# anands-repo/hello

Hardware: AMD Instinct MI355X
Metric: candidate sites/sec (whole node) (higher is better)
Workload: dtype f32

## Files before the change

### hello_amd/csrc/engine.hip

```cpp
#include <hip/hip_runtime.h>

#include <cstdarg>
#include <cstdio>
#include <cstring>
#include <new>
#include <stdexcept>
#include <string>
#include <vector>

#include "../../include/hello_mi355x.h"
#include "kernels.h"

namespace {

thread_local std::string g_last_error;

int fail(int code, const char* fmt, ...) {
    char buf[512];
    va_list ap;
    va_start(ap, fmt);
    vsnprintf(buf, sizeof(buf), fmt, ap);
    va_end(ap);
    g_last_error = buf;
    return code;
}

// ... 108 lines not shown
    bool timed = false;
    bool profiling = false;
    std::vector<std::vector<hipEvent_t>> prof_events;
    int prof_count = 0;
    int prof_filter = 0;
    int debug_op = -1;
    DevBuf d_debug;
    size_t debug_floats = 0;
    int stamp_mode = 0;
    DevBuf d_stamps;
    int32_t stamp_layout[5] = {0, 0, 0, 0, 0};

    int32_t *roff0 = nullptr, *roff1 = nullptr, *aoff = nullptr, *site_of_allele = nullptr;
    int32_t *allele_of_read0 = nullptr, *allele_of_read1 = nullptr;
    int32_t *group_slot0 = nullptr, *group_slot1 = nullptr, *slot_off0 = nullptr, *slot_off1 = nullptr;
    hello::ReadConvPlan plan0{1, 0, 0}, plan1{1, 0, 0};
    bool wide_trunk[2] = {false, false};
    int64_t* pair_off = nullptr;
};

namespace {

long long rows_of(int domain, int32_t S, int32_t A, int64_t R0, int64_t R1) {
    switch (domain) {
        case HELLO_ROWS_READS0: return R0;
        case HELLO_ROWS_READS1: return R1;
        case HELLO_ROWS_ALLELES: return A;
        case HELLO_ROWS_SITES: return S;
    }
    return -1;
}
// ... 341 lines not shown
            delete e;
            return fail(HELLO_ERR_MODEL, "a weight block runs past the end of the blob");
        }
    }
    e->scratch.resize(desc->n_buffers);
    hipError_t err = hipMalloc((void**)&e->d_weights, nbytes);
    if (err == hipSuccess) err = hipMemcpy(e->d_weights, folded_weights, nbytes, hipMemcpyHostToDevice);
    if (err == hipSuccess) err = hipStreamCreateWithFlags(&e->own_stream, hipStreamNonBlocking);
    if (err == hipSuccess) err = hipEventCreateWithFlags(&e->ev_staged, hipEventDisableTiming);
    if (err == hipSuccess) err = hipEventCreate(&e->ev_start);
    if (err == hipSuccess) err = hipEventCreate(&e->ev_stop);
    if (err != hipSuccess) {
        hello_engine_destroy(e);
        return fail(HELLO_ERR_HIP, "engine setup failed: %s", hipGetErrorString(err));
    }
    const int n_ops = (int)e->ops.size();
    e->n_lanes = lanes.n_lanes;
    e->partial_of.assign(n_ops, -1);
    int n_partial = e->n_lanes > 1 ? 0 : 2;
    for (int i = 0; i < n_ops; ++i)
        if (e->ops[i].kind == HELLO_OP_READCONV_FUSED)
            e->partial_of[i] = e->n_lanes > 1 ? n_partial++ : (e->ops[i].seg == HELLO_SEG_READS1_TO_ALLELES ? 1 : 0);
    e->d_partial.resize(n_partial);
    if (e->n_lanes > 1) {
        auto lane_of = [&](int i) { return lane_of_op(e->ops[i]); };
        e->op_waits = std::move(lanes.op_waits);
        e->lane_tail = std::move(lanes.lane_tail);
        const std::vector<char>& read_elsewhere = lanes.read_elsewhere;
        e->op_done.assign(n_ops, nullptr);
        e->lane_streams.assign(e->n_lanes, nullptr);
// ... 156 lines not shown
    HIP_TRY(hipSetDevice(e->device));
    HIP_TRY(hipStreamSynchronize(e->last_stream ? e->last_stream : e->own_stream));
    HIP_TRY(hipMemcpy(out, e->d_debug.p, e->debug_floats * sizeof(float), hipMemcpyDeviceToHost));
    return HELLO_OK;
} catch (...) {
    return hello::exception_status("hello_engine_debug_read");
}

static int stage_batch_indices(hello_engine* e, const int32_t* rpa0, const int32_t* rpa1,
                               const int32_t* aps, int32_t S, int32_t A, int64_t R0, int64_t R1,
                               bool two_tech, hipStream_t stream) {
    const int win = hello::readconv_supports_window(e->desc.window) ? e->desc.window : 150;
    const int G = hello::readconv_reads_per_group(win);
    if ((e->wide_trunk[0] || e->wide_trunk[1]) && hello::readconv_wide_reads_per_group() != G)
        return fail(HELLO_ERR_ARG, "internal: the wide trunk's group size differs from the read convolver's");
    const hello::ReadConvPlan plan0 = e->wide_trunk[0] ? hello::readconv_wide_plan(R0) : hello::readconv_plan(R0, win);
    const hello::ReadConvPlan plan1 = !two_tech ? hello::ReadConvPlan{1, 0, 0}
                                      : e->wide_trunk[1] ? hello::readconv_wide_plan(R1) : hello::readconv_plan(R1, win);
    const int64_t n_groups0 = plan0.bulk_wgs + plan0.rest_wgs, n_groups1 = plan1.bulk_wgs + plan1.rest_wgs;
    e->plan0 = plan0;
    e->plan1 = plan1;
    size_t bytes = 0;
    auto add = [&](size_t count, size_t elem) { bytes += (count * elem + 15) & ~size_t(15); };
    add(A + 1, 4); add(A + 1, 4); add(S + 1, 4); add(A, 4);
    add(R0, 4); add(R1, 4);
    add(n_groups0 + 1, 4); add(n_groups1 + 1, 4);
    add(A + 1, 4); add(A + 1, 4);
    add(S + 1, 8);
    if (e->staged_pending) {
        HIP_TRY(hipEventSynchronize(e->ev_staged));
        e->staged_pending = false;
    }
    if (e->h_csr.ensure(bytes)) return fail(HELLO_ERR_HIP, "pinned allocation of %zu bytes failed", bytes);
    if (bytes > e->d_csr.cap) {
        HIP_TRY(hipStreamSynchronize(stream));
        if (e->d_csr.ensure(bytes)) return fail(HELLO_ERR_HIP, "device allocation of %zu bytes failed", bytes);
    }
    char* hc = (char*)e->h_csr.p;
    char* hbase = hc;
    int32_t* h_roff0 = carve<int32_t>(hc, A + 1);
    int32_t* h_roff1 = carve<int32_t>(hc, A + 1);
    int32_t* h_aoff = carve<int32_t>(hc, S + 1);
    int32_t* h_soa = carve<int32_t>(hc, A);
    int32_t* h_aor0 = carve<int32_t>(hc, R0);
    int32_t* h_aor1 = carve<int32_t>(hc, R1);
    int32_t* h_gs0 = carve<int32_t>(hc, n_groups0 + 1);
    int32_t* h_gs1 = carve<int32_t>(hc, n_groups1 + 1);
    int32_t* h_so0 = carve<int32_t>(hc, A + 1);
    int32_t* h_so1 = carve<int32_t>(hc, A + 1);
    int64_t* h_poff = carve<int64_t>(hc, S + 1);

    auto build_reads = [&](const int32_t* rpa, int64_t R, int32_t* roff, int32_t* aor, int32_t* gslot,
                           int32_t* soff, const hello::ReadConvPlan& plan, const char* which) -> int {
        int64_t acc = 0;
        for (int32_t a = 0; a < A; ++a) {
            if (rpa[a] <= 0)
                return fail(HELLO_ERR_SHAPE, "%s[%d] = %d: every allele needs >= 1 read (dummy zero read)",
                            which, a, rpa[a]);
            roff[a] = (int32_t)acc;
            for (int32_t r = 0; r < rpa[a]; ++r) {
                if (acc + r < R) aor[acc + r] = a;
            }
            acc += rpa[a];
            if (acc > R) return fail(HELLO_ERR_SHAPE, "sum(%s) exceeds n_reads = %lld", which, (long long)R);
        }
        roff[A] = (int32_t)acc;
        if (acc != R)
            return fail(HELLO_ERR_SHAPE, "sum(%s) = %lld != n_reads = %lld", which, (long long)acc, (long long)R);
        const int64_t n_wgs = plan.bulk_wgs + plan.rest_wgs;
        const int64_t bulk_reads = plan.rest_wgs ? plan.bulk_wgs * plan.groups_per_wg * G : R;
        for (int32_t a = 0; a <= A; ++a) soff[a] = 0;
        int64_t slot = 0;
        for (int64_t w = 0; w < n_wgs; ++w) {
            int64_t r_lo, r_hi;
            if (w < plan.bulk_wgs) {
                r_lo = w * plan.groups_per_wg * G;
                r_hi = r_lo + (int64_t)plan.groups_per_wg * G;
                if (r_hi > bulk_reads) r_hi = bulk_reads;
            } else {
                r_lo = bulk_reads + (w - plan.bulk_wgs) * G;
                r_hi = r_lo + G < R ? r_lo + G : R;
            }
            if (r_lo >= r_hi) return fail(HELLO_ERR_ARG, "internal: empty workgroup in the read-convolver plan");
            gslot[w] = (int32_t)slot;
            const int32_t first = aor[r_lo], last = aor[r_hi - 1];
            for (int32_t a = first; a <= last; ++a) soff[a + 1] += 1;
            slot += (last - first + 1);
        }
        gslot[n_wgs] = (int32_t)slot;
        int64_t s = 0;
        for (int32_t a = 0; a < A; ++a) {
            const int32_t count = soff[a + 1];
            soff[a] = (int32_t)s;
            s += count;
        }
        soff[A] = (int32_t)s;
        if (s != slot) return fail(HELLO_ERR_ARG, "internal: slot accounting mismatch");
        return 0;
    };
    if (int rc = build_reads(rpa0, R0, h_roff0, h_aor0, h_gs0, h_so0, plan0, "reads_per_allele0")) return rc;
    if (two_tech) {
        if (int rc = build_reads(rpa1, R1, h_roff1, h_aor1, h_gs1, h_so1, plan1, "reads_per_allele1")) return rc;
    } else {
        h_gs1[0] = 0;
    }
    int64_t acc = 0, pacc = 0;
    for (int32_t s = 0; s < S; ++s) {
        if (aps[s] <= 0) return fail(HELLO_ERR_SHAPE, "alleles_per_site[%d] = %d", s, aps[s]);
        h_aoff[s] = (int32_t)acc;
        h_poff[s] = pacc;
        for (int32_t k = 0; k < aps[s] && acc + k < A; ++k) h_soa[acc + k] = s;
        acc += aps[s];
        pacc += (int64_t)aps[s] * (aps[s] + 1) / 2;
        if (acc > A) return fail(HELLO_ERR_SHAPE, "sum(alleles_per_site) exceeds n_alleles = %d", A);
    }
    h_aoff[S] = (int32_t)acc;
    h_poff[S] = pacc;
    if (acc != A) return fail(HELLO_ERR_SHAPE, "sum(alleles_per_site) = %lld != n_alleles = %d", (long long)acc, A);

    HIP_TRY(hipMemcpyAsync(e->d_csr.p, hbase, bytes, hipMemcpyHostToDevice, stream));
    HIP_TRY(hipEventRecord(e->ev_staged, stream));
    e->staged_pending = true;
    char* dbase = (char*)e->d_csr.p;
    auto dev = [&](void* hp) { return dbase + ((char*)hp - hbase); };
    e->roff0 = (int32_t*)dev(h_roff0);
    e->roff1 = (int32_t*)dev(h_roff1);
    e->aoff = (int32_t*)dev(h_aoff);
    e->site_of_allele = (int32_t*)dev(h_soa);
    e->allele_of_read0 = (int32_t*)dev(h_aor0);
    e->allele_of_read1 = (int32_t*)dev(h_aor1);
    e->group_slot0 = (int32_t*)dev(h_gs0);
    e->group_slot1 = (int32_t*)dev(h_gs1);
    e->slot_off0 = (int32_t*)dev(h_so0);
    e->slot_off1 = (int32_t*)dev(h_so1);
    e->pair_off = (int64_t*)dev(h_poff);
    return 0;
}

int hello_engine_forward(hello_engine* e, const uint8_t* reads0, const int32_t* rpa0,
                         const uint8_t* reads1, const int32_t* rpa1, const int32_t* aps,
                         const uint8_t* ref_onehot, int32_t S, int32_t A, int64_t R0, int64_t R1,
                         float* logits, float* meta, float* posteriors, int32_t flags, void* hip_stream) try {
    if (!e) return fail(HELLO_ERR_ARG, "engine is NULL");
    const hello_model_desc& d = e->desc;
    const bool two_tech = d.channels1 > 0;
    if (S <= 0 || A <= 0 || R0 <= 0) return fail(HELLO_ERR_ARG, "empty batch (S=%d A=%d R0=%lld)", S, A, (long long)R0);
    if (A < S) return fail(HELLO_ERR_SHAPE, "n_alleles %d < n_sites %d", A, S);
// ... 258 lines not shown
                a.w = e->d_weights + o.w_off;
                a.partial = (float*)e->d_partial[e->partial_of[op_index]].p;
                a.allele_of_read = t1 ? e->allele_of_read1 : e->allele_of_read0;
                a.slot_of_group = t1 ? e->group_slot1 : e->group_slot0;
                a.n_reads = t1 ? R1 : R0;
                a.window = d.window;
                a.softplus = (o.flags & HELLO_FLAG_SOFTPLUS) ? 1 : 0;
                a.extra_blocks = o.k;
                a.winograd = (o.flags & HELLO_FLAG_WINOGRAD) ? 1 : 0;
                a.bf16x3 = (o.flags & HELLO_FLAG_BF16X3) ? ((o.flags & HELLO_FLAG_BF16X3_32) ? 2 : 1) : 0;
                const bool wide = o.cout == 128;
                if ((size_t)o.w_off + (wide ? hello::readconv_wide_weight_floats() : hello::readconv_weight_floats(o.k, a.winograd, d.window)) +
                        (a.bf16x3 ? hello::readconv_bf16x3_extra_floats(o.k) : 0) > e->n_weight_floats)
                    return fail(HELLO_ERR_MODEL, "op %d: fused read-convolver weight block truncated", op_index);
                {
                    const hello::ReadConvPlan& plan = t1 ? e->plan1 : e->plan0;
                    const int G = hello::readconv_reads_per_group(d.window);
                    const long long total = a.n_reads;
                    const long long bulk_reads = plan.rest_wgs ? plan.bulk_wgs * plan.groups_per_wg * G : total;
                    a.groups_per_wg = plan.groups_per_wg;
                    a.n_reads = bulk_reads;
                    int32_t stamp_lay[5] = {0, 0, 0, 0, 0};
                    const int stamp_waves = hello::readconv_stamp_waves();
                    if ((e->stamp_mode & 1) && !t1 && total > 0) {
                        if (wide || !a.reads) return fail(HELLO_ERR_ARG, "stamps: the canonical fused read convolver from the bytes only");
                        const long long wgs = plan.rest_wgs ? plan.bulk_wgs + plan.rest_wgs : (long long)((total + (long long)G * plan.groups_per_wg - 1) / ((long long)G * plan.groups_per_wg));
                        const int slots = hello::readconv_stamp_slots();
                        const size_t bytes = (size_t)wgs * stamp_waves * plan.groups_per_wg * slots * sizeof(uint64_t);
                        if (bytes > e->d_stamps.cap) {
                            HIP_TRY(hipStreamSynchronize(stream));
                            if (e->d_stamps.ensure(bytes)) return fail(HELLO_ERR_HIP, "device allocation of %zu bytes failed", bytes);
                        }
                        HIP_TRY(hipMemsetAsync(e->d_stamps.p, 0, bytes, stream));
                        a.stamps = (unsigned long long*)e->d_stamps.p;
                        a.stamp_groups = plan.groups_per_wg;
                        a.stamp_mode = e->stamp_mode;
                        const int32_t lay[5] = {(int32_t)wgs, stamp_waves, plan.groups_per_wg, slots, (int32_t)(plan.rest_wgs ? plan.bulk_wgs : wgs)};
                        for (int i = 0; i < 5; ++i) stamp_lay[i] = lay[i];
                        e->stamp_layout[0] = 0;
                    }
                    HIP_TRY(wide ? hello::launch_readconv_wide(a, stream) : hello::launch_readconv_fused(a, stream));
                    if (plan.rest_wgs) {
                        hello::ReadConvArgs b = a;
                        if (b.stamps) b.stamps += (size_t)plan.bulk_wgs * stamp_waves * plan.groups_per_wg * hello::readconv_stamp_slots();
                        if (b.reads) b.reads += bulk_reads * d.window * o.cin;
                        else b.pooled += bulk_reads * (long long)o.lin * o.cin;
                        b.allele_of_read += bulk_reads;
                        b.slot_of_group += plan.bulk_wgs;
                        b.groups_per_wg = 1;
                        b.n_reads = total - bulk_reads;
                        HIP_TRY(wide ? hello::launch_readconv_wide(b, stream) : hello::launch_readconv_fused(b, stream));
                    }
                    if (a.stamps)
                        for (int i = 0; i < 5; ++i) e->stamp_layout[i] = stamp_lay[i];
                }
                HIP_TRY(hello::launch_readconv_finalize((const float*)e->d_partial[e->partial_of[op_index]].p, t1 ? e->slot_off1 : e->slot_off0,
                                                        (float*)ptr(o.dst), A, o.lout, o.cout, stream));
                break;
            }
        }
        if (op_index == e->debug_op) {
            const size_t per_row = o.kind == HELLO_OP_CONCAT ? (size_t)o.lout * (o.cin + o.c1)
                                   : (o.kind == HELLO_OP_CONV1D || o.kind == HELLO_OP_READCONV_FUSED || o.kind == HELLO_OP_COMPRESSOR_FUSED || o.kind == HELLO_OP_XATTN_FRONT) ? (size_t)o.lout * o.cout
                                   : (o.kind == HELLO_OP_MAXPOOL ? (size_t)o.lout * o.cin : (size_t)o.lin * o.cin);
            const size_t n = (size_t)rows * per_row;
// ... 328 lines not shown
```

### hello_amd/csrc/kernels.h

```cpp
#pragma once
#include <hip/hip_runtime.h>
#include <stdint.h>

namespace hello {

int device_cus();

struct ConvArgs {
    const void* src;
    const float* src2;
    int split;
    float* dst;
    const float* res;
    const float* w;
    const float* bias;
    long long m_total;
    int lin, lout, cin, cout, k, stride, pad;
    int cin_stride;
    int groups;
    int kpad;
    int cout_pad;
    int relu;
    int src_u8;
    unsigned wino_rows;
// ... 28 lines not shown
hipError_t launch_rcl_to_rlc(const uint8_t* src, uint8_t* dst, long long rows, int len, int c,
                             hipStream_t stream);

hipError_t launch_posteriors(const float* logits, const float* meta, const int32_t* allele_off,
                             const int64_t* pair_off, int n_sites, long long n_alleles, int n_experts,
                             long long n_pairs_total, float* out, hipStream_t stream);

struct ReadConvArgs {
    const uint8_t* reads;
    const float* pooled;
    int channels;
    const float* w;
    float* partial;
    const int32_t* allele_of_read;
    const int32_t* slot_of_group;
    int groups_per_wg;
    long long n_reads;
    int extra_blocks;
    int winograd;
    int window;
    int softplus;
    int bf16x3;
    unsigned long long* stamps;
    int stamp_groups;
    int stamp_mode;
};
int readconv_stamp_slots();
int readconv_stamp_waves();
bool readconv_supports_window(int window);
int readconv_reads_per_group(int window);
int readconv_frame_rows(int window);
int readconv_groups_per_workgroup(long long n_reads, int window);
struct ReadConvPlan {
    int groups_per_wg;
    long long bulk_wgs;
    long long rest_wgs;
};
ReadConvPlan readconv_plan(long long n_reads, int window);
ReadConvPlan readconv_wide_plan(long long n_reads);
int readconv_weight_floats(int extra_blocks, bool winograd, int window);
int readconv_bf16x3_extra_floats(int extra_blocks);
bool readconv_supports_extra_blocks(int extra_blocks);
hipError_t launch_readconv_fused(const ReadConvArgs& a, hipStream_t stream);
hipError_t launch_readconv_finalize(const float* partial, const int32_t* slot_off, float* frames, int n_alleles,
                                    int frame_rows, int channels, hipStream_t stream);
int readconv_wide_weight_floats();
int readconv_wide_reads_per_group();
hipError_t launch_readconv_wide(const ReadConvArgs& a, hipStream_t stream);

struct CompressorArgs {
    const float* frames;
    float* dst;
    const float* w;
    long long n_items;
// ... 74 lines not shown
```

### hello_amd/csrc/readconv_fused.hip

```cpp
#include <cstdlib>
#include <type_traits>

#include "kernels.h"

namespace hello {

typedef float f32x4 __attribute__((ext_vector_type(4)));

namespace rc {

constexpr int S1_STEPS = 6;
template <bool WINO, bool F33 = false>
struct Offs {
    static constexpr int KT = WINO ? 4 : 3;
    static constexpr int W3232 = 2 * KT * 2 * 256, W3264 = 4 * 3 * 2 * 256, W3264S = 4 * 1 * 2 * 256;
    static constexpr int W6464 = 4 * KT * 4 * 256;
    static constexpr int W6464D = F33 ? 4 * 5 * 4 * 256 : W6464;
    static constexpr int W3232D = F33 ? 2 * 5 * 2 * 256 : W3232;
    static constexpr int OFF_B = 0;
    static constexpr int OFF_C1 = OFF_B + 6 * (W3232D + 32);
    static constexpr int OFF_SC = OFF_C1 + W3264 + 64;
    static constexpr int OFF_C2 = OFF_SC + W3264S + 64;
    static constexpr int OFF_D = OFF_C2 + W6464D + 64;
    static constexpr int W_TRUNK = OFF_D + 6 * (W6464D + 64);
// ... 52 lines not shown
using GeometrySoftplus = rc::Cfg<4, 4, 150, rc::ACT_SOFTPLUS>;
static_assert(Geometry::F33 && GeometrySoftplus::F33 && !Geometry250::F33, "weight packing rule of readconv_pack.py");
static_assert(Geometry::F33_32 && GeometrySoftplus::F33_32, "weight packing rule of readconv_pack.py");
int readconv_bf16x3_extra_floats(int extra_blocks) { return (1 + 2 * (3 + extra_blocks)) * 12288 + 6 * 3072; }
int readconv_weight_floats(int extra_blocks, bool winograd, int window) {
    if (!winograd) return rc::Offs<false>::off_d(3 + extra_blocks);
    return window == 150 ? rc::Offs<true, true>::off_d(3 + extra_blocks) : rc::Offs<true>::off_d(3 + extra_blocks);
}
bool readconv_supports_extra_blocks(int extra_blocks) { return extra_blocks == 0 || extra_blocks == 2; }

bool readconv_supports_window(int window) { return window == 150 || window == 250; }
int readconv_reads_per_group(int window) { return window == 250 ? Geometry250::G : Geometry::G; }
int readconv_stamp_slots() { return rc::STAMP_SLOTS; }
int readconv_stamp_waves() { return Geometry::NW; }
int readconv_frame_rows(int window) { return window == 250 ? Geometry250::L2 : Geometry::L2; }
int readconv_groups_per_workgroup(long long n_reads, int window) {
    const long long slots = 2LL * device_cus();
    const int G = readconv_reads_per_group(window);
    const long long groups = (n_reads + G - 1) / G;
    int best = 1;
    double best_cost = 1e300;
    for (int n = 1; n <= 8; ++n) {
        const long long wgs = (groups + n - 1) / n;
        const double cost = (double)((wgs + slots - 1) / slots) * n * (n > 1 ? 0.988 : 1.0);
        if (cost <= best_cost) {
            best_cost = cost;
            best = n;
        }
    }
    return best;
}

ReadConvPlan readconv_plan(long long n_reads, int window) {
    const long long slots = 2LL * device_cus();
    const int G = readconv_reads_per_group(window);
    const long long groups = (n_reads + G - 1) / G;
    ReadConvPlan best{1, groups, 0};
    double best_cost = 1e300;
    for (int n = 1; n <= 8; ++n) {
        const long long rounds = (groups / n) / slots;
        if (rounds == 0) continue;
        const long long bulk = rounds * slots, rest = groups - bulk * n;
        const double cost = (double)rounds * n * (n > 1 ? 0.988 : 1.0) + (double)((rest + slots - 1) / slots);
        if (cost <= best_cost) {
            best_cost = cost;
            best = ReadConvPlan{n, bulk, rest};
        }
    }
    if (best_cost == 1e300) {
        const int n = readconv_groups_per_workgroup(n_reads, window);
        best = ReadConvPlan{n, (groups + n - 1) / n, 0};
    }
    return best;
}

template <int C>
__device__ __forceinline__ int swz(int row) {
    return (C == 64 || C == 128) ? 2 * (row & 7) : (C == 32 ? 2 * ((row >> 1) & 3) : 2 * ((row >> 2) & 1));
}

enum { SW_OLD = 0, SW_W = 1, SW_3 = 2, SW_SPLIT = 3, SW_GLOBAL = 4 };

typedef short bf16x8 __attribute__((ext_vector_type(8)));
typedef short bf16x4 __attribute__((ext_vector_type(4)));
__device__ __forceinline__ int split_off(int row, int g, int part) { return row * 256 + 16 * ((g + 8 * part) ^ (2 * (row & 7))); }
__device__ __forceinline__ unsigned short to_bf16(float x) {
    const __bf16 h = (__bf16)x;
    return __builtin_bit_cast(unsigned short, h);
}
// ... 1016 lines not shown
            }
        } else {
#pragma unroll
            for (int k = 0; k < T1 / 2; ++k) pad1 |= ((((pg1 + 2 * k) * 16 + j) % RS1) >= L1 ? 1u : 0u) << k;
        }
    }

    float* const X = STEM ? bufB : bufA;
    float* const H = STEM ? bufA : bufB;
    f32x4 sreg[CF::NSREG];
    f32x4 wA[NVA], wB[NVB], w2[2];
    f32x4 w3[2][5];
    f32x4 (&w6)[6] = reinterpret_cast<f32x4 (&)[6]>(wA);
    f32x4 (&w12)[12] = reinterpret_cast<f32x4 (&)[12]>(wB);

    const long long wg_read0 = (long long)blockIdx.x * G * a.groups_per_wg;
    const int slot0 = a.slot_of_group[blockIdx.x];
    const int first_allele = a.allele_of_read[wg_read0];
    int cur = first_allele;
    constexpr int NF = (L2 * 16 + THREADS - 1) / THREADS;
    f32x4 carry[NF];
#pragma unroll
    for (int i = 0; i < NF; ++i) carry[i] = f32x4{0.f, 0.f, 0.f, 0.f};
    auto flush = [&]() {
#pragma unroll
        for (int i = 0; i < NF; ++i) {
            const int f = tid0 + THREADS * i;
            if (f < L2 * 16)
                *(f32x4*)(a.partial + ((long long)(slot0 + cur - first_allele) * L2 + (f >> 4)) * 64 + 4 * (f & 15)) = carry[i];
            carry[i] = f32x4{0.f, 0.f, 0.f, 0.f};
        }
    };

    for (int grp = 0; grp < a.groups_per_wg; ++grp) {
    int opaque_zero;
    asm volatile("s_mov_b32 %0, 0" : "=s"(opaque_zero));
    const int tid = tid0 + opaque_zero;
    const int wave = __builtin_amdgcn_readfirstlane(wave0 + opaque_zero);
    const int lane = tid & 63;
    const int cb2 = wave % 2, cb4 = wave;
    const long long read0 = wg_read0 + (long long)grp * G;
    if (read0 >= a.n_reads) break;
    unsigned long long* const stamp_base = STAMP ? a.stamps + (((long long)blockIdx.x * CF::NW + wave) * a.stamp_groups + grp) * STAMP_SLOTS : nullptr;
    auto stamp = [&](int slot) {
        if constexpr (STAMP) {
            const unsigned long long t = __builtin_amdgcn_s_memtime();
            if (grp < a.stamp_groups && lane == 0) stamp_base[slot] = t;
        }
    };
    auto barrier = [&](int id) {
        stamp(1 + 2 * id);
        __syncthreads();
        stamp(2 + 2 * id);
    };
    if constexpr (STAMP) {
        stamp(0);
        const unsigned long long rt = __builtin_amdgcn_s_memrealtime();
        const unsigned hw = __builtin_amdgcn_s_getreg((31 << 11) | 4), xcc = __builtin_amdgcn_s_getreg((31 << 11) | 20);
// ... 254 lines not shown
#pragma unroll
                for (int e = 0; e < 4; ++e) carry[i][e] += v[e];
            }
        }
    }
    barrier(19);
    if constexpr (STAMP) {
        const unsigned long long rt = __builtin_amdgcn_s_memrealtime();
        if (grp < a.stamp_groups && lane == 0) stamp_base[43] = rt;
    }
    }
    flush();
    if constexpr (STAMP) {
        static_assert(!STAMP || (NB64 == 3 && STEM && WINO && !BF16), "stamps: the default fp32 Winograd schedule (20 barriers per group)");
        const unsigned long long t = __builtin_amdgcn_s_memtime();
        if ((tid0 & 63) == 0) a.stamps[(((long long)blockIdx.x * CF::NW + wave0) * a.stamp_groups) * STAMP_SLOTS + 44] = t;
    }
}

template <class CF, int NB64, bool WINO, bool STEM_ONLY = false, bool BF16 = false, bool BF16_32 = false>
static hipError_t launch_cfg(const ReadConvArgs& a, hipStream_t stream) {
    static bool configured_on[64] = {};
    int dev = 0;
    if (hipGetDevice(&dev) != hipSuccess || dev < 0 || dev >= 64) return hipErrorInvalidDevice;
    bool& configured = configured_on[dev];
    if (!configured) {
        hipError_t e = hipSuccess;
        if constexpr (!STEM_ONLY)
            e = hipFuncSetAttribute((const void*)readconv_kernel<CF, false, NB64, WINO, BF16, BF16_32>,
                                    hipFuncAttributeMaxDynamicSharedMemorySize, CF::LDS_BYTES);
        if (e == hipSuccess)
            e = hipFuncSetAttribute((const void*)readconv_kernel<CF, true, NB64, WINO, BF16, BF16_32>,
                                    hipFuncAttributeMaxDynamicSharedMemorySize, CF::LDS_BYTES);
        if (e != hipSuccess) return e;
        configured = true;
    }
    if (a.groups_per_wg < 1) return hipErrorInvalidValue;
    const long long per_wg = (long long)CF::G * a.groups_per_wg;
    const unsigned groups = (unsigned)((a.n_reads + per_wg - 1) / per_wg);
    if (a.stamps) {
        if constexpr (std::is_same<CF, Geometry>::value && NB64 == 3 && WINO && !BF16 && !STEM_ONLY) {
            if (!a.reads || (a.channels != 6 && a.channels != 7) || a.stamp_groups < 1) return hipErrorInvalidValue;
            static bool stamped_on[64] = {};
            if (!stamped_on[dev]) {
                const hipError_t e = hipFuncSetAttribute((const void*)readconv_kernel<CF, true, NB64, WINO, false, false, true>,
                                                         hipFuncAttributeMaxDynamicSharedMemorySize, 100 * 1024);
                if (e != hipSuccess) return e;
                stamped_on[dev] = true;
            }
            const int lds = (a.stamp_mode & 2) ? 100 * 1024 : CF::LDS_BYTES;
            hipLaunchKernelGGL((readconv_kernel<CF, true, NB64, WINO, false, false, true>), dim3(groups), dim3(CF::THREADS), lds, stream, a);
            return hipGetLastError();
        } else {
            return hipErrorInvalidValue;
// ... 487 lines not shown
#pragma unroll
        for (int b = 0; b < 2; ++b) {
            const f32x4 y0 = (a[b][0] + a[b][1]) + a[b][2];
            const f32x4 y1 = (a[b][1] - a[b][2]) - a[b][3];
            f32x4 v;
#pragma unroll
            for (int e = 0; e < 4; ++e) v[e] = CF::act(fmaxf(fmaxf(y0[e], y1[e]), row_shl(y0[e], 1)));
            float* ptr = out + img_off<64, SW_3>(1 + rd * CF::RS1 + pos, 4 * (2 * half + b) + q);
            *(f32x4*)(ok ? ptr : dump) = v;
        }
    });
}

int readconv_wide_weight_floats() { return wt::Cfg::W_TOTAL; }
int readconv_wide_reads_per_group() { return wt::Cfg::G; }
ReadConvPlan readconv_wide_plan(long long n_reads) {
    return ReadConvPlan{1, (n_reads + wt::Cfg::G - 1) / wt::Cfg::G, 0};
}

template <bool STEM>
__global__ __launch_bounds__(wt::Cfg::THREADS, 2) void readconv_wide_kernel(ReadConvArgs a) {
    using CF = wt::Cfg;
    constexpr int G = CF::G, L1 = CF::L1, RS1 = CF::RS1, L2 = CF::L2, THREADS = CF::THREADS;
    extern __shared__ __attribute__((aligned(16))) float smem[];
    float* const X = smem;
    float* const H = smem + CF::BUF_FLOATS;
    int* const s_allele = (int*)(smem + 2 * CF::BUF_FLOATS);
    float* const dump = smem + 2 * CF::BUF_FLOATS + 12;
    const int tid0 = threadIdx.x;
    const int wave0 = __builtin_amdgcn_readfirstlane(tid0 >> 6);
    const float* __restrict__ W = a.w;
    const f32x4 zero4 = {0.f, 0.f, 0.f, 0.f};

    const int tid = tid0, wave = wave0, lane = tid0 & 63;
    const int cb4 = wave % 4;
    const long long read0 = (long long)blockIdx.x * G;
    const int n_here = (int)((a.n_reads - read0) < G ? (a.n_reads - read0) : G);
    f32x4 w3[2][5];
    auto slice64 = [&](int off) { return W + off + cb4 * (4 * 5 * 256) + lane * 4; };
    auto slice128 = [&](int off) { return W + off + wave * (8 * 5 * 256) + lane * 4; };
#pragma unroll
    for (int c = 0; c < 5; ++c) w3[0][c] = *(const f32x4*)(slice64(CF::off_a(0)) + c * 256);
    if (tid < G) s_allele[tid] = (tid < n_here) ? a.allele_of_read[read0 + tid] : -1;
    if constexpr (STEM) {
        unsigned char* const s_u8 = (unsigned char*)(smem + 2 * CF::BUF_FLOATS + 16);
        const int ch = a.channels;
        const int n_bytes = n_here * CF::WINDOW * ch;
        const unsigned char* src = a.reads + read0 * CF::WINDOW * ch;
        constexpr int NDW = (CF::U8_BYTES / 4 + THREADS - 1) / THREADS;
        if ((reinterpret_cast<unsigned long long>(src) & 3ull) == 0) {
            unsigned v[NDW];
// ... 101 lines not shown
        int oz;
        asm volatile("s_mov_b32 %0, 0" : "=s"(oz));
        const int lane_b = lane + oz, wave_b = __builtin_amdgcn_readfirstlane(wave + oz);
        auto slice = [&](int off) { return W + off + wave_b * (8 * 5 * 256) + lane_b * 4; };
        const int off_a = CF::off_b(1 + 2 * blk), off_b = CF::off_b(2 + 2 * blk);
        wino3_layer<CF, 128, MODE_PLAIN, false, L2>(H, X, w3, slice(off_a), slice(off_b), W + off_a + CF::WB, wave_b, lane_b);
        __syncthreads();
        if (blk < 2)
            wino3_layer<CF, 128, MODE_RESID_INPLACE, false, L2>(X, H, w3, slice(off_b), slice(CF::off_b(3 + 2 * blk)),
                                                                W + off_b + CF::WB, wave_b, lane_b);
        else
            wino3_layer<CF, 128, MODE_RESID_INPLACE, true, L2>(X, H, w3, slice(off_b), nullptr, W + off_b + CF::WB, wave_b, lane_b);
        __syncthreads();
    }

    const int slot0 = a.slot_of_group[blockIdx.x];
    const int first_allele = s_allele[0];
    int cur = first_allele;
    constexpr int NF = (L2 * 32 + THREADS - 1) / THREADS;
    f32x4 carry[NF];
#pragma unroll
    for (int i = 0; i < NF; ++i) carry[i] = zero4;
    auto flush = [&]() {
#pragma unroll
        for (int i = 0; i < NF; ++i) {
            const int f = tid + THREADS * i;
            if (f < L2 * 32)
                *(f32x4*)(a.partial + ((long long)(slot0 + cur - first_allele) * L2 + (f >> 5)) * 128 + 4 * (f & 31)) = carry[i];
            carry[i] = zero4;
        }
    };
// ... 7 lines not shown
        for (int i = 0; i < NF; ++i) {
            const int f = tid + THREADS * i;
            if (f < L2 * 32) {
                const f32x4 v = *(const f32x4*)(H + img_off<128, SW_3>(1 + rd * L2 + (f >> 5), f & 31));
#pragma unroll
                for (int e = 0; e < 4; ++e) carry[i][e] += v[e];
            }
        }
    }
    flush();
}

hipError_t launch_readconv_wide(const ReadConvArgs& a, hipStream_t stream) {
    if (a.n_reads <= 0) return hipSuccess;
    if ((!a.pooled == !a.reads) || !a.w || !a.partial || !a.winograd || a.window != 150 || a.extra_blocks != 0 || a.softplus ||
        a.groups_per_wg != 1 || (a.reads && a.channels != 6 && a.channels != 7))
        return hipErrorInvalidValue;
    static bool configured_on[64] = {};
    int dev = 0;
    if (hipGetDevice(&dev) != hipSuccess || dev < 0 || dev >= 64) return hipErrorInvalidDevice;
    if (!configured_on[dev]) {
        hipError_t e = hipFuncSetAttribute((const void*)readconv_wide_kernel<false>, hipFuncAttributeMaxDynamicSharedMemorySize,
                                           wt::Cfg::LDS_BYTES);
        if (e == hipSuccess)
            e = hipFuncSetAttribute((const void*)readconv_wide_kernel<true>, hipFuncAttributeMaxDynamicSharedMemorySize, wt::Cfg::LDS_BYTES);
        if (e != hipSuccess) return e;
        configured_on[dev] = true;
    }
    const unsigned grid = (unsigned)((a.n_reads + wt::Cfg::G - 1) / wt::Cfg::G);
    if (a.reads) hipLaunchKernelGGL(readconv_wide_kernel<true>, dim3(grid), dim3(wt::Cfg::THREADS), wt::Cfg::LDS_BYTES, stream, a);
    else hipLaunchKernelGGL(readconv_wide_kernel<false>, dim3(grid), dim3(wt::Cfg::THREADS), wt::Cfg::LDS_BYTES, stream, a);
    return hipGetLastError();
}

}
```

Before: 488,300.

## Replace bulk/rest read-convolver plan with a tapered per-workgroup group worklist

Workgroups now look up a first_group table instead of using a fixed groups_per_wg, so one launch can hand out chunks of 8, 4, 2 and 1 read groups per workgroup. Large chunks go first and small ones last, which shrinks the tail and replaces the previous two-launch bulk/rest scheme as the default. This is meant to cut tail imbalance and the second kernel launch. The cost is an extra staged index array and an indirect load per workgroup, and the old plan stays reachable through an environment variable.

Result: no change. 490,300, median of 6 (+0.4%).

```diff
diff --git a/hello_amd/csrc/engine.hip b/hello_amd/csrc/engine.hip
--- a/hello_amd/csrc/engine.hip
+++ b/hello_amd/csrc/engine.hip
@@ -2,6 +2,7 @@
 
 #include <cstdarg>
 #include <cstdio>
+#include <cstdlib>
 #include <cstring>
 #include <new>
 #include <stdexcept>
@@ -10,6 +11,7 @@
 
 #include "../../include/hello_mi355x.h"
 #include "kernels.h"
+#include "readconv_worklist.h"
 
 namespace {
 
@@ -148,7 +150,14 @@
     int32_t *roff0 = nullptr, *roff1 = nullptr, *aoff = nullptr, *site_of_allele = nullptr;
     int32_t *allele_of_read0 = nullptr, *allele_of_read1 = nullptr;
     int32_t *group_slot0 = nullptr, *group_slot1 = nullptr, *slot_off0 = nullptr, *slot_off1 = nullptr;
-    hello::ReadConvPlan plan0{1, 0, 0}, plan1{1, 0, 0};
+    int32_t *first_group0 = nullptr, *first_group1 = nullptr;
+    struct WorkList {
+        std::vector<int32_t> first_group;
+        long long first_launch = 0;
+        long long n_wgs() const { return (long long)first_group.size() - 1; }
+    } worklist[2];
+    bool two_launch = false;
+    hello::ReadConvTaper taper = hello::READCONV_TAPER_DEFAULT;
     bool wide_trunk[2] = {false, false};
     int64_t* pair_off = nullptr;
 };
@@ -520,6 +529,17 @@
         hello_engine_destroy(e);
         return fail(HELLO_ERR_HIP, "engine setup failed: %s", hipGetErrorString(err));
     }
+    if (const char* plan = std::getenv("HELLO_READCONV_PLAN")) {
+        int t[3];
+        if (!strcmp(plan, "two-launch")) {
+            e->two_launch = true;
+        } else if (sscanf(plan, "tapered:%d,%d,%d", &t[0], &t[1], &t[2]) == 3 && t[0] >= 0 && t[1] >= 0 && t[2] >= 0 && t[0] <= 1024 && t[1] <= 1024 && t[2] <= 1024) {
+            e->taper = hello::ReadConvTaper{{t[0], t[1], t[2]}};
+        } else if (strcmp(plan, "tapered") && plan[0]) {
+            hello_engine_destroy(e);
+            return fail(HELLO_ERR_ARG, "HELLO_READCONV_PLAN=%s: two-launch | tapered | tapered:a,b,c", plan);
+        }
+    }
     const int n_ops = (int)e->ops.size();
     e->n_lanes = lanes.n_lanes;
     e->partial_of.assign(n_ops, -1);
@@ -706,16 +726,23 @@
     const int G = hello::readconv_reads_per_group(win);
     if ((e->wide_trunk[0] || e->wide_trunk[1]) && hello::readconv_wide_reads_per_group() != G)
         return fail(HELLO_ERR_ARG, "internal: the wide trunk's group size differs from the read convolver's");
-    const hello::ReadConvPlan plan0 = e->wide_trunk[0] ? hello::readconv_wide_plan(R0) : hello::readconv_plan(R0, win);
-    const hello::ReadConvPlan plan1 = !two_tech ? hello::ReadConvPlan{1, 0, 0}
-                                      : e->wide_trunk[1] ? hello::readconv_wide_plan(R1) : hello::readconv_plan(R1, win);
-    const int64_t n_groups0 = plan0.bulk_wgs + plan0.rest_wgs, n_groups1 = plan1.bulk_wgs + plan1.rest_wgs;
-    e->plan0 = plan0;
-    e->plan1 = plan1;
+    const long long slots = hello::readconv_resident_slots();
+    auto plan = [&](int t, int64_t R) {
+        hello_engine::WorkList& wl = e->worklist[t];
+        const long long groups = (R + G - 1) / G;
+        if (e->wide_trunk[t]) hello::readconv_worklist_uniform(groups, 1, wl.first_group);
+        else if (e->two_launch) wl.first_launch = hello::readconv_worklist_bulk_rest(groups, slots, wl.first_group);
+        else hello::readconv_worklist_tapered(groups, slots, e->taper, wl.first_group);
+        if (e->wide_trunk[t] || !e->two_launch) wl.first_launch = wl.n_wgs();
+    };
+    plan(0, R0);
+    plan(1, two_tech ? R1 : 0);
+    const int64_t n_groups0 = e->worklist[0].n_wgs(), n_groups1 = e->worklist[1].n_wgs();
     size_t bytes = 0;
     auto add = [&](size_t count, size_t elem) { bytes += (count * elem + 15) & ~size_t(15); };
     add(A + 1, 4); add(A + 1, 4); add(S + 1, 4); add(A, 4);
     add(R0, 4); add(R1, 4);
+    add(n_groups0 + 1, 4); add(n_groups1 + 1, 4);
     add(n_groups0 + 1, 4); add(n_groups1 + 1, 4);
     add(A + 1, 4); add(A + 1, 4);
     add(S + 1, 8);
@@ -738,12 +765,16 @@
     int32_t* h_aor1 = carve<int32_t>(hc, R1);
     int32_t* h_gs0 = carve<int32_t>(hc, n_groups0 + 1);
     int32_t* h_gs1 = carve<int32_t>(hc, n_groups1 + 1);
+    int32_t* h_fg0 = carve<int32_t>(hc, n_groups0 + 1);
+    int32_t* h_fg1 = carve<int32_t>(hc, n_groups1 + 1);
+    memcpy(h_fg0, e->worklist[0].first_group.data(), (size_t)(n_groups0 + 1) * sizeof(int32_t));
+    memcpy(h_fg1, e->worklist[1].first_group.data(), (size_t)(n_groups1 + 1) * sizeof(int32_t));
     int32_t* h_so0 = carve<int32_t>(hc, A + 1);
     int32_t* h_so1 = carve<int32_t>(hc, A + 1);
     int64_t* h_poff = carve<int64_t>(hc, S + 1);
 
     auto build_reads = [&](const int32_t* rpa, int64_t R, int32_t* roff, int32_t* aor, int32_t* gslot,
-                           int32_t* soff, const hello::ReadConvPlan& plan, const char* which) -> int {
+                           int32_t* soff, const std::vector<int32_t>& first_group, const char* which) -> int {
         int64_t acc = 0;
         for (int32_t a = 0; a < A; ++a) {
             if (rpa[a] <= 0)
@@ -759,40 +790,13 @@
         roff[A] = (int32_t)acc;
         if (acc != R)
             return fail(HELLO_ERR_SHAPE, "sum(%s) = %lld != n_reads = %lld", which, (long long)acc, (long long)R);
-        const int64_t n_wgs = plan.bulk_wgs + plan.rest_wgs;
-        const int64_t bulk_reads = plan.rest_wgs ? plan.bulk_wgs * plan.groups_per_wg * G : R;
-        for (int32_t a = 0; a <= A; ++a) soff[a] = 0;
-        int64_t slot = 0;
-        for (int64_t w = 0; w < n_wgs; ++w) {
-            int64_t r_lo, r_hi;
-            if (w < plan.bulk_wgs) {
-                r_lo = w * plan.groups_per_wg * G;
-                r_hi = r_lo + (int64_t)plan.groups_per_wg * G;
-                if (r_hi > bulk_reads) r_hi = bulk_reads;
-            } else {
-                r_lo = bulk_reads + (w - plan.bulk_wgs) * G;
-                r_hi = r_lo + G < R ? r_lo + G : R;
-            }
-            if (r_lo >= r_hi) return fail(HELLO_ERR_ARG, "internal: empty workgroup in the read-convolver plan");
-            gslot[w] = (int32_t)slot;
-            const int32_t first = aor[r_lo], last = aor[r_hi - 1];
-            for (int32_t a = first; a <= last; ++a) soff[a + 1] += 1;
-            slot += (last - first + 1);
-        }
-        gslot[n_wgs] = (int32_t)slot;
-        int64_t s = 0;
-        for (int32_t a = 0; a < A; ++a) {
-            const int32_t count = soff[a + 1];
-            soff[a] = (int32_t)s;
-            s += count;
-        }
-        soff[A] = (int32_t)s;
-        if (s != slot) return fail(HELLO_ERR_ARG, "internal: slot accounting mismatch");
+        if (hello::readconv_number_slots(first_group.data(), (long long)first_group.size() - 1, G, R, aor, A, gslot, soff) < 0)
+            return fail(HELLO_ERR_ARG, "internal: the read convolver's work list has an empty workgroup or its slots do not add up");
         return 0;
     };
-    if (int rc = build_reads(rpa0, R0, h_roff0, h_aor0, h_gs0, h_so0, plan0, "reads_per_allele0")) return rc;
+    if (int rc = build_reads(rpa0, R0, h_roff0, h_aor0, h_gs0, h_so0, e->worklist[0].first_group, "reads_per_allele0")) return rc;
     if (two_tech) {
-        if (int rc = build_reads(rpa1, R1, h_roff1, h_aor1, h_gs1, h_so1, plan1, "reads_per_allele1")) return rc;
+        if (int rc = build_reads(rpa1, R1, h_roff1, h_aor1, h_gs1, h_so1, e->worklist[1].first_group, "reads_per_allele1")) return rc;
     } else {
         h_gs1[0] = 0;
     }
@@ -823,6 +827,8 @@
     e->allele_of_read1 = (int32_t*)dev(h_aor1);
     e->group_slot0 = (int32_t*)dev(h_gs0);
     e->group_slot1 = (int32_t*)dev(h_gs1);
+    e->first_group0 = (int32_t*)dev(h_fg0);
+    e->first_group1 = (int32_t*)dev(h_fg1);
     e->slot_off0 = (int32_t*)dev(h_so0);
     e->slot_off1 = (int32_t*)dev(h_so1);
     e->pair_off = (int64_t*)dev(h_poff);
@@ -1111,41 +1117,39 @@
                         (a.bf16x3 ? hello::readconv_bf16x3_extra_floats(o.k) : 0) > e->n_weight_floats)
                     return fail(HELLO_ERR_MODEL, "op %d: fused read-convolver weight block truncated", op_index);
                 {
-                    const hello::ReadConvPlan& plan = t1 ? e->plan1 : e->plan0;
-                    const int G = hello::readconv_reads_per_group(d.window);
-                    const long long total = a.n_reads;
-                    const long long bulk_reads = plan.rest_wgs ? plan.bulk_wgs * plan.groups_per_wg * G : total;
-                    a.groups_per_wg = plan.groups_per_wg;
-                    a.n_reads = bulk_reads;
+                    const hello_engine::WorkList& wl = e->worklist[t1 ? 1 : 0];
+                    const long long wgs = wl.n_wgs();
+                    a.first_group = t1 ? e->first_group1 : e->first_group0;
+                    a.wg_base = 0;
+                    a.n_wgs = (int)wl.first_launch;
                     int32_t stamp_lay[5] = {0, 0, 0, 0, 0};
-                    const int stamp_waves = hello::readconv_stamp_waves();
-                    if ((e->stamp_mode & 1) && !t1 && total > 0) {
+                    if ((e->stamp_mode & 1) && !t1 && wgs > 0) {
                         if (wide || !a.reads) return fail(HELLO_ERR_ARG, "stamps: the canonical fused read convolver from the bytes only");
-                        const long long wgs = plan.rest_wgs ? plan.bulk_wgs + plan.rest_wgs : (long long)((total + (long long)G * plan.groups_per_wg - 1) / ((long long)G * plan.groups_per_wg));
-                        const int slots = hello::readconv_stamp_slots();
-                        const size_t bytes = (size_t)wgs * stamp_waves * plan.groups_per_wg * slots * sizeof(uint64_t);
+                        const std::vector<int32_t>& fg = wl.first_group;
+                        int most = 1;
+                        for (long long w = 0; w < wgs; ++w) most = fg[w + 1] - fg[w] > most ? fg[w + 1] - fg[w] : most;
+                        long long bulk = wgs;
+                        while (bulk > 0 && fg[bulk] - fg[bulk - 1] == 1) --bulk;
+                        if (bulk == 0) bulk = wgs;
+                        const int stamp_waves = hello::readconv_stamp_waves(), slots = hello::readconv_stamp_slots();
+                        const size_t bytes = (size_t)wgs * stamp_waves * most * slots * sizeof(uint64_t);
                         if (bytes > e->d_stamps.cap) {
                             HIP_TRY(hipStreamSynchronize(stream));
                             if (e->d_stamps.ensure(bytes)) return fail(HELLO_ERR_HIP, "device allocation of %zu bytes failed", bytes);
                         }
                         HIP_TRY(hipMemsetAsync(e->d_stamps.p, 0, bytes, stream));
                         a.stamps = (unsigned long long*)e->d_stamps.p;
-                        a.stamp_groups = plan.groups_per_wg;
+                        a.stamp_groups = most;
                         a.stamp_mode = e->stamp_mode;
-                        const int32_t lay[5] = {(int32_t)wgs, stamp_waves, plan.groups_per_wg, slots, (int32_t)(plan.rest_wgs ? plan.bulk_wgs : wgs)};
+                        const int32_t lay[5] = {(int32_t)wgs, stamp_waves, most, slots, (int32_t)bulk};
                         for (int i = 0; i < 5; ++i) stamp_lay[i] = lay[i];
                         e->stamp_layout[0] = 0;
                     }
-                    HIP_TRY(wide ? hello::launch_readconv_wide(a, stream) : hello::launch_readconv_fused(a, stream));
-                    if (plan.rest_wgs) {
+                    if (a.n_wgs > 0) HIP_TRY(wide ? hello::launch_readconv_wide(a, stream) : hello::launch_readconv_fused(a, stream));
+                    if (wl.first_launch < wgs) {
                         hello::ReadConvArgs b = a;
-                        if (b.stamps) b.stamps += (size_t)plan.bulk_wgs * stamp_waves * plan.groups_per_wg * hello::readconv_stamp_slots();
-                        if (b.reads) b.reads += bulk_reads * d.window * o.cin;
-                        else b.pooled += bulk_reads * (long long)o.lin * o.cin;
-                        b.allele_of_read += bulk_reads;
-                        b.slot_of_group += plan.bulk_wgs;
-                        b.groups_per_wg = 1;
-                        b.n_reads = total - bulk_reads;
+                        b.wg_base = (int)wl.first_launch;
+                        b.n_wgs = (int)(wgs - wl.first_launch);
                         HIP_TRY(wide ? hello::launch_readconv_wide(b, stream) : hello::launch_readconv_fused(b, stream));
                     }
                     if (a.stamps)
diff --git a/hello_amd/csrc/kernels.h b/hello_amd/csrc/kernels.h
--- a/hello_amd/csrc/kernels.h
+++ b/hello_amd/csrc/kernels.h
@@ -66,7 +66,9 @@
     float* partial;
     const int32_t* allele_of_read;
     const int32_t* slot_of_group;
-    int groups_per_wg;
+    const int32_t* first_group;
+    int wg_base;
+    int n_wgs;
     long long n_reads;
     int extra_blocks;
     int winograd;
@@ -82,14 +84,7 @@
 bool readconv_supports_window(int window);
 int readconv_reads_per_group(int window);
 int readconv_frame_rows(int window);
-int readconv_groups_per_workgroup(long long n_reads, int window);
-struct ReadConvPlan {
-    int groups_per_wg;
-    long long bulk_wgs;
-    long long rest_wgs;
-};
-ReadConvPlan readconv_plan(long long n_reads, int window);
-ReadConvPlan readconv_wide_plan(long long n_reads);
+long long readconv_resident_slots();
 int readconv_weight_floats(int extra_blocks, bool winograd, int window);
 int readconv_bf16x3_extra_floats(int extra_blocks);
 bool readconv_supports_extra_blocks(int extra_blocks);
diff --git a/hello_amd/csrc/readconv_fused.hip b/hello_amd/csrc/readconv_fused.hip
--- a/hello_amd/csrc/readconv_fused.hip
+++ b/hello_amd/csrc/readconv_fused.hip
@@ -90,45 +90,7 @@
 int readconv_stamp_slots() { return rc::STAMP_SLOTS; }
 int readconv_stamp_waves() { return Geometry::NW; }
 int readconv_frame_rows(int window) { return window == 250 ? Geometry250::L2 : Geometry::L2; }
-int readconv_groups_per_workgroup(long long n_reads, int window) {
-    const long long slots = 2LL * device_cus();
-    const int G = readconv_reads_per_group(window);
-    const long long groups = (n_reads + G - 1) / G;
-    int best = 1;
-    double best_cost = 1e300;
-    for (int n = 1; n <= 8; ++n) {
-        const long long wgs = (groups + n - 1) / n;
-        const double cost = (double)((wgs + slots - 1) / slots) * n * (n > 1 ? 0.988 : 1.0);
-        if (cost <= best_cost) {
-            best_cost = cost;
-            best = n;
-        }
-    }
-    return best;
-}
-
-ReadConvPlan readconv_plan(long long n_reads, int window) {
-    const long long slots = 2LL * device_cus();
-    const int G = readconv_reads_per_group(window);
-    const long long groups = (n_reads + G - 1) / G;
-    ReadConvPlan best{1, groups, 0};
-    double best_cost = 1e300;
-    for (int n = 1; n <= 8; ++n) {
-        const long long rounds = (groups / n) / slots;
-        if (rounds == 0) continue;
-        const long long bulk = rounds * slots, rest = groups - bulk * n;
-        const double cost = (double)rounds * n * (n > 1 ? 0.988 : 1.0) + (double)((rest + slots - 1) / slots);
-        if (cost <= best_cost) {
-            best_cost = cost;
-            best = ReadConvPlan{n, bulk, rest};
-        }
-    }
-    if (best_cost == 1e300) {
-        const int n = readconv_groups_per_workgroup(n_reads, window);
-        best = ReadConvPlan{n, (groups + n - 1) / n, 0};
-    }
-    return best;
-}
+long long readconv_resident_slots() { return 2LL * device_cus(); }
 
 template <int C>
 __device__ __forceinline__ int swz(int row) {
@@ -1175,8 +1137,10 @@
     f32x4 (&w6)[6] = reinterpret_cast<f32x4 (&)[6]>(wA);
     f32x4 (&w12)[12] = reinterpret_cast<f32x4 (&)[12]>(wB);
 
-    const long long wg_read0 = (long long)blockIdx.x * G * a.groups_per_wg;
-    const int slot0 = a.slot_of_group[blockIdx.x];
+    const int wg = blockIdx.x + a.wg_base;
+    const int group0 = a.first_group[wg], n_groups = a.first_group[wg + 1] - group0;
+    const long long wg_read0 = (long long)group0 * G;
+    const int slot0 = a.slot_of_group[wg];
     const int first_allele = a.allele_of_read[wg_read0];
     int cur = first_allele;
     constexpr int NF = (L2 * 16 + THREADS - 1) / THREADS;
@@ -1193,7 +1157,7 @@
         }
     };
 
-    for (int grp = 0; grp < a.groups_per_wg; ++grp) {
+    for (int grp = 0; grp < n_groups; ++grp) {
     int opaque_zero;
     asm volatile("s_mov_b32 %0, 0" : "=s"(opaque_zero));
     const int tid = tid0 + opaque_zero;
@@ -1202,7 +1166,7 @@
     const int cb2 = wave % 2, cb4 = wave;
     const long long read0 = wg_read0 + (long long)grp * G;
     if (read0 >= a.n_reads) break;
-    unsigned long long* const stamp_base = STAMP ? a.stamps + (((long long)blockIdx.x * CF::NW + wave) * a.stamp_groups + grp) * STAMP_SLOTS : nullptr;
+    unsigned long long* const stamp_base = STAMP ? a.stamps + (((long long)wg * CF::NW + wave) * a.stamp_groups + grp) * STAMP_SLOTS : nullptr;
     auto stamp = [&](int slot) {
         if constexpr (STAMP) {
             const unsigned long long t = __builtin_amdgcn_s_memtime();
@@ -1487,7 +1451,7 @@
     if constexpr (STAMP) {
         static_assert(!STAMP || (NB64 == 3 && STEM && WINO && !BF16), "stamps: the default fp32 Winograd schedule (20 barriers per group)");
         const unsigned long long t = __builtin_amdgcn_s_memtime();
-        if ((tid0 & 63) == 0) a.stamps[(((long long)blockIdx.x * CF::NW + wave0) * a.stamp_groups) * STAMP_SLOTS + 44] = t;
+        if ((tid0 & 63) == 0) a.stamps[(((long long)wg * CF::NW + wave0) * a.stamp_groups) * STAMP_SLOTS + 44] = t;
     }
 }
 
@@ -1508,9 +1472,9 @@
         if (e != hipSuccess) return e;
         configured = true;
     }
-    if (a.groups_per_wg < 1) return hipErrorInvalidValue;
-    const long long per_wg = (long long)CF::G * a.groups_per_wg;
-    const unsigned groups = (unsigned)((a.n_reads + per_wg - 1) / per_wg);
+    if (!a.first_group || a.n_wgs < 1 || a.wg_base < 0) return hipErrorInvalidValue;
+    if ((long long)a.wg_base + a.n_wgs > (a.n_reads + CF::G - 1) / CF::G) return hipErrorInvalidValue;
+    const unsigned groups = (unsigned)a.n_wgs;
     if (a.stamps) {
         if constexpr (std::is_same<CF, Geometry>::value && NB64 == 3 && WINO && !BF16 && !STEM_ONLY) {
             if (!a.reads || (a.channels != 6 && a.channels != 7) || a.stamp_groups < 1) return hipErrorInvalidValue;
@@ -2028,9 +1992,6 @@
 
 int readconv_wide_weight_floats() { return wt::Cfg::W_TOTAL; }
 int readconv_wide_reads_per_group() { return wt::Cfg::G; }
-ReadConvPlan readconv_wide_plan(long long n_reads) {
-    return ReadConvPlan{1, (n_reads + wt::Cfg::G - 1) / wt::Cfg::G, 0};
-}
 
 template <bool STEM>
 __global__ __launch_bounds__(wt::Cfg::THREADS, 2) void readconv_wide_kernel(ReadConvArgs a) {
@@ -2048,7 +2009,8 @@
 
     const int tid = tid0, wave = wave0, lane = tid0 & 63;
     const int cb4 = wave % 4;
-    const long long read0 = (long long)blockIdx.x * G;
+    const int wg = blockIdx.x + a.wg_base;
+    const long long read0 = (long long)a.first_group[wg] * G;
     const int n_here = (int)((a.n_reads - read0) < G ? (a.n_reads - read0) : G);
     f32x4 w3[2][5];
     auto slice64 = [&](int off) { return W + off + cb4 * (4 * 5 * 256) + lane * 4; };
@@ -2180,7 +2142,7 @@
         __syncthreads();
     }
 
-    const int slot0 = a.slot_of_group[blockIdx.x];
+    const int slot0 = a.slot_of_group[wg];
     const int first_allele = s_allele[0];
     int cur = first_allele;
     constexpr int NF = (L2 * 32 + THREADS - 1) / THREADS;
@@ -2218,8 +2180,9 @@
 hipError_t launch_readconv_wide(const ReadConvArgs& a, hipStream_t stream) {
     if (a.n_reads <= 0) return hipSuccess;
     if ((!a.pooled == !a.reads) || !a.w || !a.partial || !a.winograd || a.window != 150 || a.extra_blocks != 0 || a.softplus ||
-        a.groups_per_wg != 1 || (a.reads && a.channels != 6 && a.channels != 7))
+        !a.first_group || a.n_wgs < 1 || a.wg_base < 0 || (a.reads && a.channels != 6 && a.channels != 7))
         return hipErrorInvalidValue;
+    if ((long long)a.wg_base + a.n_wgs > (a.n_reads + wt::Cfg::G - 1) / wt::Cfg::G) return hipErrorInvalidValue;
     static bool configured_on[64] = {};
     int dev = 0;
     if (hipGetDevice(&dev) != hipSuccess || dev < 0 || dev >= 64) return hipErrorInvalidDevice;
@@ -2231,7 +2194,7 @@
         if (e != hipSuccess) return e;
         configured_on[dev] = true;
     }
-    const unsigned grid = (unsigned)((a.n_reads + wt::Cfg::G - 1) / wt::Cfg::G);
+    const unsigned grid = (unsigned)a.n_wgs;
     if (a.reads) hipLaunchKernelGGL(readconv_wide_kernel<true>, dim3(grid), dim3(wt::Cfg::THREADS), wt::Cfg::LDS_BYTES, stream, a);
     else hipLaunchKernelGGL(readconv_wide_kernel<false>, dim3(grid), dim3(wt::Cfg::THREADS), wt::Cfg::LDS_BYTES, stream, a);
     return hipGetLastError();
diff --git a/hello_amd/csrc/readconv_worklist.h b/hello_amd/csrc/readconv_worklist.h
--- /dev/null
+++ b/hello_amd/csrc/readconv_worklist.h
@@ -0,0 +1,124 @@
+#pragma once
+#include <stdint.h>
+
+#include <vector>
+
+namespace hello {
+
+constexpr int READCONV_MOST_GROUPS = 8;
+
+inline int readconv_single_launch_groups(long long groups, long long slots) {
+    int best = 1;
+    double best_cost = 1e300;
+    for (int n = 1; n <= READCONV_MOST_GROUPS; ++n) {
+        const long long wgs = (groups + n - 1) / n;
+        const double cost = (double)((wgs + slots - 1) / slots) * n * (n > 1 ? 0.988 : 1.0);
+        if (cost <= best_cost) {
+            best_cost = cost;
+            best = n;
+        }
+    }
+    return best;
+}
+
+struct ReadConvBulkRest {
+    int n;
+    long long bulk, rest;
+};
+inline ReadConvBulkRest readconv_bulk_rest(long long groups, long long slots) {
+    ReadConvBulkRest best{1, groups, 0};
+    double best_cost = 1e300;
+    for (int n = 1; n <= READCONV_MOST_GROUPS; ++n) {
+        const long long rounds = (groups / n) / slots;
+        if (rounds == 0) continue;
+        const long long bulk = rounds * slots, rest = groups - bulk * n;
+        const double cost = (double)rounds * n * (n > 1 ? 0.988 : 1.0) + (double)((rest + slots - 1) / slots);
+        if (cost <= best_cost) {
+            best_cost = cost;
+            best = ReadConvBulkRest{n, bulk, rest};
+        }
+    }
+    if (best_cost == 1e300) {
+        const int n = readconv_single_launch_groups(groups, slots);
+        best = ReadConvBulkRest{n, (groups + n - 1) / n, 0};
+    }
+    return best;
+}
+
+inline void readconv_worklist_append(std::vector<int32_t>& first_group, long long count, int n, long long groups) {
+    long long g = first_group.back();
+    for (long long i = 0; i < count && g < groups; ++i) {
+        g = g + n < groups ? g + n : groups;
+        first_group.push_back((int32_t)g);
+    }
+}
+
+inline void readconv_worklist_uniform(long long groups, int n, std::vector<int32_t>& first_group) {
+    first_group.assign(1, 0);
+    readconv_worklist_append(first_group, (groups + n - 1) / n, n, groups);
+}
+
+inline long long readconv_worklist_bulk_rest(long long groups, long long slots, std::vector<int32_t>& first_group) {
+    const ReadConvBulkRest p = readconv_bulk_rest(groups, slots);
+    first_group.assign(1, 0);
+    readconv_worklist_append(first_group, p.bulk, p.n, groups);
+    readconv_worklist_append(first_group, p.rest, 1, groups);
+    return p.bulk;
+}
+
+struct ReadConvTaper {
+    int per64[3];
+};
+constexpr ReadConvTaper READCONV_TAPER_DEFAULT{{64, 64, 64}};
+
+inline void readconv_worklist_tapered(long long groups, long long slots, const ReadConvTaper& taper, std::vector<int32_t>& first_group) {
+    if (groups < slots) {
+        readconv_worklist_uniform(groups, readconv_single_launch_groups(groups, slots), first_group);
+        return;
+    }
+    long long left = groups, count[4] = {0, 0, 0, 0};
+    const long long want1 = slots * taper.per64[2] / 64;
+    count[3] = left < want1 ? left : want1;
+    left -= count[3];
+    for (int ph = 2; ph >= 0; --ph) {
+        const int n = 8 >> ph;
+        long long c = left / n;
+        if (ph > 0) {
+            const long long want = slots * taper.per64[ph - 1] / 64;
+            if (c > want) c = want;
+        }
+        c -= c % 8;
+        count[ph] = c;
+        left -= c * n;
+    }
+    count[3] += left;
+    first_group.assign(1, 0);
+    for (int ph = 0; ph < 4; ++ph) readconv_worklist_append(first_group, count[ph], 8 >> ph, groups);
+}
+
+inline long long readconv_number_slots(const int32_t* first_group, long long n_wgs, int G, long long n_reads,
+                                       const int32_t* allele_of_read, int32_t n_alleles, int32_t* wg_slot, int32_t* allele_slot) {
+    for (int32_t a = 0; a <= n_alleles; ++a) allele_slot[a] = 0;
+    long long slot = 0;
+    for (long long w = 0; w < n_wgs; ++w) {
+        const long long r_lo = (long long)first_group[w] * G;
+        long long r_hi = (long long)first_group[w + 1] * G;
+        if (r_hi > n_reads) r_hi = n_reads;
+        if (r_lo < 0 || r_lo >= r_hi) return -1;
+        wg_slot[w] = (int32_t)slot;
+        const int32_t first = allele_of_read[r_lo], last = allele_of_read[r_hi - 1];
+        for (int32_t a = first; a <= last; ++a) allele_slot[a + 1] += 1;
+        slot += last - first + 1;
+    }
+    wg_slot[n_wgs] = (int32_t)slot;
+    long long s = 0;
+    for (int32_t a = 0; a < n_alleles; ++a) {
+        const int32_t count = allele_slot[a + 1];
+        allele_slot[a] = (int32_t)s;
+        s += count;
+    }
+    allele_slot[n_alleles] = (int32_t)s;
+    return s == slot ? slot : -1;
+}
+
+}
```
